# tensorlink-lab/tensorlink

Hardware: NVIDIA H100
Metric: generate tokens/sec (higher is better)
Workload: dtype bf16

## Files before the change

tensorlink_b200/csrc/attention.cu:

```cuda
#include <stdlib.h>

#include "common.cuh"

namespace tl {

constexpr int FA_BQ = 64, FA_BKV = 64, FA_THREADS = 128;

__device__ __forceinline__ void cp_async16(void* smem_dst, const void* gsrc, bool valid) {
    const uint32_t d = smem_u32(smem_dst);
    const int sz = valid ? 16 : 0;
    asm volatile("cp.async.cg.shared.global [%0], [%1], 16, %2;" ::"r"(d), "l"(gsrc), "r"(sz) : "memory");
}
__device__ __forceinline__ void cp_async_commit() { asm volatile("cp.async.commit_group;" ::: "memory"); }
template <int N>
__device__ __forceinline__ void cp_async_wait() { asm volatile("cp.async.wait_group %0;" ::"n"(N) : "memory"); }

__device__ __forceinline__ void ldmatrix_x4(uint32_t* r, const void* p) {
    asm volatile("ldmatrix.sync.aligned.m8n8.x4.shared.b16 {%0,%1,%2,%3}, [%4];"
                 : "=r"(r[0]), "=r"(r[1]), "=r"(r[2]), "=r"(r[3]) : "r"(smem_u32(p)));
}
__device__ __forceinline__ void ldmatrix_x4_trans(uint32_t* r, const void* p) {
    asm volatile("ldmatrix.sync.aligned.m8n8.x4.trans.shared.b16 {%0,%1,%2,%3}, [%4];"
                 : "=r"(r[0]), "=r"(r[1]), "=r"(r[2]), "=r"(r[3]) : "r"(smem_u32(p)));
}
// ... 584 lines not shown
                for (int ks = 0; ks < D / 16; ++ks)
                    ldmatrix_x4(qf[ks], sQ + (warp * 16 + (lane & 15)) * LDS + ks * 16 + (lane >> 4) * 8);
            }
            const bf16* sKb = sK + (t & 1) * FA_BKV * LDS;
            const bf16* sVb = sV + (t & 1) * FA_BKV * LDS;
            float s[FA_BKV / 8][4];
#pragma unroll
            for (int i = 0; i < FA_BKV / 8; ++i) s[i][0] = s[i][1] = s[i][2] = s[i][3] = 0.f;
#pragma unroll
            for (int ks = 0; ks < D / 16; ++ks) {
#pragma unroll
                for (int np = 0; np < FA_BKV / 16; ++np) {
                    uint32_t bfr[4];
                    const int mi = lane >> 3;
                    ldmatrix_x4(bfr, sKb + (np * 16 + (mi >> 1) * 8 + (lane & 7)) * LDS + ks * 16 + (mi & 1) * 8);
                    mma_bf16_16816(s[2 * np], qf[ks], bfr[0], bfr[1]);
                    mma_bf16_16816(s[2 * np + 1], qf[ks], bfr[2], bfr[3]);
                }
            }
            const int kv0 = c0 + t * FA_BKV;
            float mx[2] = {-INFINITY, -INFINITY};
#pragma unroll
            for (int i = 0; i < FA_BKV / 8; ++i) {
#pragma unroll
                for (int e = 0; e < 4; ++e) {
                    const int key = kv0 + i * 8 + 2 * t4 + (e & 1);
                    const float v = key <= last[e >> 1] ? s[i][e] * scale_log2 : -INFINITY;
                    s[i][e] = v;
                    mx[e >> 1] = fmaxf(mx[e >> 1], v);
                }
            }
            float alpha[2], msub[2];
#pragma unroll
            for (int r = 0; r < 2; ++r) {
                mx[r] = fmaxf(mx[r], __shfl_xor_sync(0xffffffffu, mx[r], 1));
                mx[r] = fmaxf(mx[r], __shfl_xor_sync(0xffffffffu, mx[r], 2));
                const float m_new = fmaxf(m_run[r], mx[r]);
                msub[r] = (m_new == -INFINITY) ? 0.f : m_new;
                alpha[r] = exp2f(m_run[r] - msub[r]);
                m_run[r] = m_new;
            }
            float rs[2] = {0.f, 0.f};
            uint32_t pf[FA_BKV / 16][4];
#pragma unroll
            for (int i = 0; i < FA_BKV / 8; ++i) {
                const float p0 = exp2f(s[i][0] - msub[0]), p1 = exp2f(s[i][1] - msub[0]);
                const float p2 = exp2f(s[i][2] - msub[1]), p3 = exp2f(s[i][3] - msub[1]);
                rs[0] += p0 + p1;
                rs[1] += p2 + p3;
                pf[i >> 1][(i & 1) * 2] = pack_bf16(p0, p1);
                pf[i >> 1][(i & 1) * 2 + 1] = pack_bf16(p2, p3);
            }
#pragma unroll
            for (int r = 0; r < 2; ++r) {
                rs[r] += __shfl_xor_sync(0xffffffffu, rs[r], 1);
                rs[r] += __shfl_xor_sync(0xffffffffu, rs[r], 2);
                l_run[r] = l_run[r] * alpha[r] + rs[r];
            }
#pragma unroll
            for (int i = 0; i < D / 8; ++i) {
                o[i][0] *= alpha[0];
                o[i][1] *= alpha[0];
                o[i][2] *= alpha[1];
                o[i][3] *= alpha[1];
            }
#pragma unroll
            for (int kk = 0; kk < FA_BKV / 16; ++kk) {
#pragma unroll
                for (int dp = 0; dp < D / 16; ++dp) {
                    uint32_t bfr[4];
                    const int mi = lane >> 3;
                    ldmatrix_x4_trans(bfr, sVb + (kk * 16 + (mi & 1) * 8 + (lane & 7)) * LDS + dp * 16 + (mi >> 1) * 8);
                    mma_bf16_16816(o[2 * dp], pf[kk], bfr[0], bfr[1]);
                    mma_bf16_16816(o[2 * dp + 1], pf[kk], bfr[2], bfr[3]);
                }
            }
        }
        if (t + 2 < n_tiles) {
            __syncthreads();
            load_tile(t + 2);
        }
    }
    if (!active) return;
#pragma unroll
    for (int r = 0; r < 2; ++r) {
        const int m = m0 + warp * 16 + g + r * 8;
        if (m >= M) continue;
        float* rec = ws + (((size_t)kvh * n_splits + split) * M + m) * (2 + D);
        if (t4 == 0) { rec[0] = m_run[r]; rec[1] = l_run[r]; }
#pragma unroll
        for (int i = 0; i < D / 8; ++i)
            *reinterpret_cast<float2*>(rec + 2 + i * 8 + 2 * t4) = make_float2(o[i][2 * r], o[i][2 * r + 1]);
    }
}

template <int D>
__global__ void attn_verify_reduce_kernel(const float* __restrict__ ws, bf16* __restrict__ out, const int32_t* __restrict__ pos_dev,
                                          int q_len, int n_h, int n_kv, int T_max, int n_splits) {
    const int h = blockIdx.x, i = blockIdx.y, dd = threadIdx.x;
    const int n_rep = n_h / n_kv, kvh = h / n_rep, M = n_rep * q_len, m = i * n_rep + (h - kvh * n_rep);
    const int last = min(*pos_dev + i, T_max - 1);
    const int ns = min(n_splits, last / DEC_CHUNK_MMA + 1);
    const float* base = ws + ((size_t)kvh * n_splits * M + m) * (2 + D);
    const size_t step = (size_t)M * (2 + D);
    float Mx = -INFINITY;
    for (int s = 0; s < ns; ++s) Mx = fmaxf(Mx, base[s * step]);
    float L = 0.f, O = 0.f;
    for (int s = 0; s < ns; ++s) {
        const float* rec = base + s * step;
        if (rec[0] == -INFINITY) continue;
        const float w = exp2f(rec[0] - Mx);
        L += rec[1] * w;
        O += rec[2 + dd] * w;
    }
    out[((size_t)i * n_h + h) * D + dd] = f2bf(L > 0.f ? O / L : 0.f);
}

}

namespace tl {
int attn_prefill_wgmma(const void* q, const void* k_cache, const void* v_cache, void* out, float* lse, int B, int S, int past_len,
                       int n_h, int n_kv, int d, int T_max, float scale, const int32_t* kv_start, cudaStream_t st);

static int attn_prefill_launch(const void* q, const void* k_cache, const void* v_cache, void* out, float* lse, int B, int S,
                               int past_len, int n_h, int n_kv, int d, int T_max, float scale, const int32_t* kv_start,
                               cudaStream_t st, const char* what) {
    TL_REQUIRE(d == 64 || d == 128, TL_ERR_INVALID, "%s: head_dim %d not in {64,128}", what, d);
    TL_REQUIRE(n_kv > 0 && n_h % n_kv == 0, TL_ERR_INVALID, "%s: n_h %% n_kv != 0", what);
    TL_REQUIRE(past_len >= 0 && past_len + S <= T_max, TL_ERR_INVALID,
               "%s: past_len %d + S %d exceeds cache T_max %d", what, past_len, S, T_max);
    if (B == 0 || S == 0) return TL_OK;
    {
        const char* e = getenv("TL_ATTN_IMPL");
        const int impl = !e ? 0 : (e[0] == 'm' ? 1 : (e[0] == 'w' ? 2 : 0));
        if (impl == 2 || (impl == 0 && S >= FA_BQ))
            return attn_prefill_wgmma(q, k_cache, v_cache, out, lse, B, S, past_len, n_h, n_kv, d, T_max, scale, kv_start, st);
    }
    const dim3 grid((S + FA_BQ - 1) / FA_BQ, n_h, B);
    const float sl2 = scale * 1.4426950408889634f;
    const size_t smem = (size_t)(FA_BQ + 4 * FA_BKV) * (d + 8) * sizeof(bf16);
#define TL_FA_FWD(D_, ROWS_)                                                                                                \
    do {                                                                                                                    \
        static bool done = false;                                                                                           \
        if (!done) { cudaFuncSetAttribute(attn_prefill_kernel<D_, ROWS_>, cudaFuncAttributeMaxDynamicSharedMemorySize, (int)smem); done = true; } \
        attn_prefill_kernel<D_, ROWS_><<<grid, FA_THREADS, smem, st>>>((const bf16*)q, (const bf16*)k_cache, (const bf16*)v_cache, \
                                                                        (bf16*)out, lse, S, past_len, n_h, n_kv, T_max, sl2, kv_start); \
    } while (0)
    if (kv_start) {
        if (d == 64) TL_FA_FWD(64, true); else TL_FA_FWD(128, true);
    } else {
        if (d == 64) TL_FA_FWD(64, false); else TL_FA_FWD(128, false);
    }
#undef TL_FA_FWD
    return check_launch(what);
}

static int attn_decode_launch(const void* q, const void* k_cache, const void* v_cache, void* out, const int32_t* kv_len_dev,
                              void* workspace, size_t ws_bytes, int B, int n_h, int n_kv, int d, int T_max, float scale,
                              const int32_t* kv_start, cudaStream_t st, const char* what);
}

extern "C" {

int tl_attn_prefill_fwd(const void* q, const void* k_cache, const void* v_cache, void* out, float* lse, int B, int S,
                        int past_len, int n_h, int n_kv, int d, int T_max, float scale, void* stream) {
    return tl::attn_prefill_launch(q, k_cache, v_cache, out, lse, B, S, past_len, n_h, n_kv, d, T_max, scale, nullptr,
                                   (cudaStream_t)stream, "tl_attn_prefill_fwd");
}

int tl_attn_prefill_fwd_rows(const void* q, const void* k_cache, const void* v_cache, void* out, float* lse, int B, int S,
                             int past_len, int n_h, int n_kv, int d, int T_max, float scale, const int32_t* kv_start_dev,
                             void* stream) {
    using namespace tl;
    TL_REQUIRE(kv_start_dev != nullptr, TL_ERR_INVALID, "tl_attn_prefill_fwd_rows: kv_start_dev is null");
    return attn_prefill_launch(q, k_cache, v_cache, out, lse, B, S, past_len, n_h, n_kv, d, T_max, scale, kv_start_dev,
                               (cudaStream_t)stream, "tl_attn_prefill_fwd_rows");
}

size_t tl_attn_decode_ws(int B, int n_h, int d, int T_max) {
    const size_t n_splits = (size_t)(T_max + tl::DEC_CHUNK - 1) / tl::DEC_CHUNK;
    return (size_t)B * n_splits * (size_t)n_h * (2 + d) * sizeof(float);
}

int tl_attn_decode_fwd(const void* q, const void* k_cache, const void* v_cache, void* out, const int32_t* kv_len_dev,
                       void* workspace, size_t ws_bytes, int B, int n_h, int n_kv, int d, int T_max, float scale,
                       void* stream) {
    return tl::attn_decode_launch(q, k_cache, v_cache, out, kv_len_dev, workspace, ws_bytes, B, n_h, n_kv, d, T_max, scale,
                                  nullptr, (cudaStream_t)stream, "tl_attn_decode_fwd");
}

int tl_attn_decode_fwd_rows(const void* q, const void* k_cache, const void* v_cache, void* out, const int32_t* kv_len_dev,
                            void* workspace, size_t ws_bytes, int B, int n_h, int n_kv, int d, int T_max, float scale,
                            const int32_t* kv_start_dev, void* stream) {
    using namespace tl;
    TL_REQUIRE(kv_start_dev != nullptr, TL_ERR_INVALID, "tl_attn_decode_fwd_rows: kv_start_dev is null");
    return attn_decode_launch(q, k_cache, v_cache, out, kv_len_dev, workspace, ws_bytes, B, n_h, n_kv, d, T_max, scale,
                              kv_start_dev, (cudaStream_t)stream, "tl_attn_decode_fwd_rows");
}

size_t tl_attn_verify_ws(int q_len, int n_h, int d, int T_max) {
    const size_t n_splits = (size_t)(T_max + tl::DEC_CHUNK_MMA - 1) / tl::DEC_CHUNK_MMA;
    return n_splits * (size_t)n_h * (size_t)(q_len > 0 ? q_len : 0) * (2 + d) * sizeof(float);
}

int tl_attn_verify_fwd(const void* q, const void* k_cache, const void* v_cache, void* out, const int32_t* pos_dev,
                       void* workspace, size_t ws_bytes, int q_len, int n_h, int n_kv, int d, int T_max, float scale,
                       void* stream) {
    using namespace tl;
    const char* what = "tl_attn_verify_fwd";
    TL_REQUIRE(d == 64 || d == 128, TL_ERR_INVALID, "%s: head_dim %d not in {64,128}", what, d);
    TL_REQUIRE(n_kv > 0 && n_h % n_kv == 0 && n_h / n_kv <= DEC_MAX_REP, TL_ERR_INVALID,
               "%s: GQA group %d/%d unsupported (max %d)", what, n_h, n_kv, DEC_MAX_REP);
    TL_REQUIRE(q_len >= 1 && q_len <= VER_MAX_Q, TL_ERR_INVALID, "%s: q_len %d not in [1, %d]", what, q_len, VER_MAX_Q);
    TL_REQUIRE(q && k_cache && v_cache && out && pos_dev && workspace, TL_ERR_INVALID, "%s: null argument", what);
    TL_REQUIRE(T_max >= q_len, TL_ERR_INVALID, "%s: T_max %d < q_len %d", what, T_max, q_len);
    TL_REQUIRE(ws_bytes >= tl_attn_verify_ws(q_len, n_h, d, T_max), TL_ERR_WORKSPACE,
               "%s: workspace %zu < %zu", what, ws_bytes, tl_attn_verify_ws(q_len, n_h, d, T_max));
    const int n_splits = (T_max + DEC_CHUNK_MMA - 1) / DEC_CHUNK_MMA;
    const int M = n_h / n_kv * q_len;
    const dim3 g1(n_splits, n_kv, (M + FA_BQ - 1) / FA_BQ), g2(n_h, q_len);
    const float sl2 = scale * 1.4426950408889634f;
    const size_t smem = (size_t)(FA_BQ + 4 * FA_BKV) * (d + 8) * sizeof(bf16);
    cudaStream_t st = (cudaStream_t)stream;
#define TL_VERIFY(D_)                                                                                                       \
    do {                                                                                                                    \
        static bool done = false;                                                                                           \
        if (!done) { cudaFuncSetAttribute(attn_verify_mma_kernel<D_>, cudaFuncAttributeMaxDynamicSharedMemorySize, (int)smem); done = true; } \
        attn_verify_mma_kernel<D_><<<g1, FA_THREADS, smem, st>>>((const bf16*)q, (const bf16*)k_cache, (const bf16*)v_cache,     \
                                                                 (float*)workspace, pos_dev, q_len, n_h, n_kv, T_max, n_splits, sl2); \
        attn_verify_reduce_kernel<D_><<<g2, D_, 0, st>>>((const float*)workspace, (bf16*)out, pos_dev, q_len, n_h, n_kv, T_max, \
                                                         n_splits);                                                         \
    } while (0)
    if (d == 64) TL_VERIFY(64); else TL_VERIFY(128);
#undef TL_VERIFY
    return check_launch(what);
}

}

namespace tl {
static int attn_decode_launch(const void* q, const void* k_cache, const void* v_cache, void* out, const int32_t* kv_len_dev,
                              void* workspace, size_t ws_bytes, int B, int n_h, int n_kv, int d, int T_max, float scale,
                              const int32_t* kv_start, cudaStream_t st, const char* what) {
    TL_REQUIRE(d == 64 || d == 128, TL_ERR_INVALID, "%s: head_dim %d not in {64,128}", what, d);
    TL_REQUIRE(n_kv > 0 && n_h % n_kv == 0 && n_h / n_kv <= DEC_MAX_REP, TL_ERR_INVALID,
               "%s: GQA group %d/%d unsupported (max %d)", what, n_h, n_kv, DEC_MAX_REP);
    TL_REQUIRE(kv_len_dev != nullptr, TL_ERR_INVALID, "%s: kv_len_dev is null", what);
    TL_REQUIRE(ws_bytes >= tl_attn_decode_ws(B, n_h, d, T_max), TL_ERR_WORKSPACE,
               "%s: workspace %zu < %zu", what, ws_bytes, tl_attn_decode_ws(B, n_h, d, T_max));
    if (B == 0) return TL_OK;
    const int n_splits = (T_max + DEC_CHUNK - 1) / DEC_CHUNK;
    const float sl2 = scale * 1.4426950408889634f;
    const dim3 g1(n_splits, n_kv, B), g2(n_h, B);
    const char* impl = getenv("TL_DECODE_ATTN");
    if (!(impl && impl[0] == 's')) {
        const int ns_m = (T_max + DEC_CHUNK_MMA - 1) / DEC_CHUNK_MMA;
        const dim3 gm(ns_m, n_kv, B);
        const size_t smem = (size_t)(16 + 4 * FA_BKV) * (d + 8) * sizeof(bf16);
#define TL_DEC_MMA(D_, ROWS_)                                                                                               \
        do {                                                                                                                \
            static bool done = false;                                                                                       \
            if (!done) { cudaFuncSetAttribute(attn_decode_mma_kernel<D_, ROWS_>, cudaFuncAttributeMaxDynamicSharedMemorySize, (int)smem); done = true; } \
            attn_decode_mma_kernel<D_, ROWS_><<<gm, FA_THREADS, smem, st>>>((const bf16*)q, (const bf16*)k_cache, (const bf16*)v_cache, \
                                                                             (float*)workspace, kv_len_dev, n_h, n_kv, T_max, ns_m, sl2, kv_start); \
            attn_decode_reduce_kernel<D_, ROWS_><<<g2, D_, 0, st>>>((const float*)workspace, (bf16*)out, kv_len_dev, n_h, n_kv, ns_m, \
                                                                     DEC_CHUNK_MMA, kv_start);                             \
        } while (0)
        if (kv_start) {
            if (d == 64) TL_DEC_MMA(64, true); else TL_DEC_MMA(128, true);
        } else {
            if (d == 64) TL_DEC_MMA(64, false); else TL_DEC_MMA(128, false);
        }
#undef TL_DEC_MMA
        return check_launch(what);
    }
#define TL_DEC_SIMT(D_, ROWS_)                                                                                              \
    do {                                                                                                                    \
        attn_decode_split_kernel<D_, ROWS_><<<g1, DEC_THREADS, 0, st>>>((const bf16*)q, (const bf16*)k_cache, (const bf16*)v_cache, \
                                                                         (float*)workspace, kv_len_dev, n_h, n_kv, T_max, n_splits, sl2, kv_start); \
        attn_decode_reduce_kernel<D_, ROWS_><<<g2, D_, 0, st>>>((const float*)workspace, (bf16*)out, kv_len_dev, n_h, n_kv, n_splits, \
                                                                 DEC_CHUNK, kv_start);                                     \
    } while (0)
    if (kv_start) {
        if (d == 64) TL_DEC_SIMT(64, true); else TL_DEC_SIMT(128, true);
    } else {
        if (d == 64) TL_DEC_SIMT(64, false); else TL_DEC_SIMT(128, false);
    }
#undef TL_DEC_SIMT
    return check_launch(what);
}
}

namespace tl {

constexpr int FD_THREADS = 128, FD_MAX_T = 2048;

template <int D, bool ROWS>
__global__ void __launch_bounds__(FD_THREADS) attn_decode_fused_kernel(
    const bf16* __restrict__ qkv, bf16* __restrict__ k_cache, bf16* __restrict__ v_cache, bf16* __restrict__ out,
    const int32_t* __restrict__ pos_dev, const bf16* __restrict__ cos_tab, const bf16* __restrict__ sin_tab,
    const bf16* __restrict__ q_norm_w, const bf16* __restrict__ k_norm_w, float eps, int n_h, int n_kv, int T_max,
    float scale_log2, const int32_t* __restrict__ kv_start) {
    constexpr int HALF = D / 2;
    asm volatile("griddepcontrol.wait;" ::: "memory");
    asm volatile("griddepcontrol.launch_dependents;");
    const int h = blockIdx.x, b = blockIdx.y, tid = threadIdx.x, lane = tid & 31, warp = tid >> 5;
    const int n_rep = n_h / n_kv, kvh = h / n_rep;
    const int pos = *pos_dev;
    int k_start = 0;
    if constexpr (ROWS) {
        k_start = kv_start[b];
        cos_tab -= (size_t)k_start * HALF;
        sin_tab -= (size_t)k_start * HALF;
    }
    const int heads = n_h + 2 * n_kv;
    __shared__ __align__(16) float sq[D], sk[D], sv[D];
    __shared__ float sscore[FD_MAX_T + 1];
    __shared__ float sred[FD_THREADS / 32];
    __shared__ float s_bc[2];
    __shared__ __align__(16) float so[FD_THREADS / 32][D];

    const bf16* row = qkv + (size_t)b * heads * D;
    float q1 = 0.f, q2 = 0.f, k1 = 0.f, k2 = 0.f;
    if (tid < HALF) {
        q1 = bf2f(row[(size_t)h * D + tid]);
        q2 = bf2f(row[(size_t)h * D + tid + HALF]);
        k1 = bf2f(row[(size_t)(n_h + kvh) * D + tid]);
        k2 = bf2f(row[(size_t)(n_h + kvh) * D + tid + HALF]);
        sv[tid] = bf2f(row[(size_t)(n_h + n_kv + kvh) * D + tid]);
        sv[tid + HALF] = bf2f(row[(size_t)(n_h + n_kv + kvh) * D + tid + HALF]);
    }
    if (q_norm_w) {
        float a = warp_sum(q1 * q1 + q2 * q2), c = warp_sum(k1 * k1 + k2 * k2);
        __shared__ float nr[2][FD_THREADS / 32];
        if (lane == 0) { nr[0][warp] = a; nr[1][warp] = c; }
        __syncthreads();
        a = c = 0.f;
#pragma unroll
        for (int w = 0; w < FD_THREADS / 32; ++w) { a += nr[0][w]; c += nr[1][w]; }
        const float rq = 1.0f / sqrtf(a / (float)D + eps), rk = 1.0f / sqrtf(c / (float)D + eps);
        if (tid < HALF) {
            q1 = rbf(bf2f(q_norm_w[tid]) * rbf(q1 * rq));
            q2 = rbf(bf2f(q_norm_w[tid + HALF]) * rbf(q2 * rq));
            k1 = rbf(bf2f(k_norm_w[tid]) * rbf(k1 * rk));
            k2 = rbf(bf2f(k_norm_w[tid + HALF]) * rbf(k2 * rk));
        }
    }
    if (tid < HALF) {
        const float c = bf2f(cos_tab[(size_t)pos * HALF + tid]), s = bf2f(sin_tab[(size_t)pos * HALF + tid]);
        sq[tid] = rbf(rbf(q1 * c) + rbf(-q2 * s));
        sq[tid + HALF] = rbf(rbf(q2 * c) + rbf(q1 * s));
        sk[tid] = rbf(rbf(k1 * c) + rbf(-k2 * s));
        sk[tid + HALF] = rbf(rbf(k2 * c) + rbf(k1 * s));
    }
    __syncthreads();
    if (h % n_rep == 0 && tid < D) {
        const size_t off = (((size_t)b * n_kv + kvh) * T_max + pos) * D + tid;
        k_cache[off] = f2bf(sk[tid]);
        v_cache[off] = f2bf(sv[tid]);
    }
    const bf16* kb = k_cache + ((size_t)b * n_kv + kvh) * T_max * D;
    const bf16* vb = v_cache + ((size_t)b * n_kv + kvh) * T_max * D;
    float mx = -INFINITY;
    for (int key = tid; key < pos; key += FD_THREADS) {
        if constexpr (ROWS) if (key < k_start) continue;
        const uint4* kr = reinterpret_cast<const uint4*>(kb + (size_t)key * D);
        float acc = 0.f;
#pragma unroll 4
        for (int c = 0; c < D / 8; ++c) {
            const uint4 kv4 = kr[c];
            const uint32_t* k32 = reinterpret_cast<const uint32_t*>(&kv4);
            const float4 qa = *reinterpret_cast<const float4*>(&sq[c * 8]);
            const float4 qb = *reinterpret_cast<const float4*>(&sq[c * 8 + 4]);
            acc += bf16_lo(k32[0]) * qa.x + bf16_hi(k32[0]) * qa.y + bf16_lo(k32[1]) * qa.z + bf16_hi(k32[1]) * qa.w +
                   bf16_lo(k32[2]) * qb.x + bf16_hi(k32[2]) * qb.y + bf16_lo(k32[3]) * qb.z + bf16_hi(k32[3]) * qb.w;
        }
        acc *= scale_log2;
        sscore[key] = acc;
        mx = fmaxf(mx, acc);
    }
    if (warp == 0) {
        float acc = 0.f;
        for (int i = lane; i < D; i += 32) acc += sq[i] * sk[i];
        acc = warp_sum(acc) * scale_log2;
        if (lane == 0) sscore[pos] = acc;
        mx = fmaxf(mx, acc);
    }
    mx = warp_max(mx);
    if (lane == 0) sred[warp] = mx;
    __syncthreads();
    if (tid == 0) {
        float m = sred[0];
#pragma unroll
        for (int w = 1; w < FD_THREADS / 32; ++w) m = fmaxf(m, sred[w]);
        s_bc[0] = m;
    }
    __syncthreads();
    const float m_all = s_bc[0];
    float lsum = 0.f;
    for (int key = tid; key <= pos; key += FD_THREADS) {
        if constexpr (ROWS) if (key < k_start) continue;
        const float p = exp2f(sscore[key] - m_all);
        lsum += p;
        sscore[key] = rbf(p);
    }
    lsum = warp_sum(lsum);
    __syncthreads();
    if (lane == 0) sred[warp] = lsum;
    __syncthreads();
    constexpr int TPR = D / 8, KG = FD_THREADS / TPR;
    const int dd0 = (tid % TPR) * 8, kgi = tid / TPR;
    float acc[8];
#pragma unroll
    for (int j = 0; j < 8; ++j) acc[j] = 0.f;
    for (int key = kgi; key < pos; key += KG) {
        if constexpr (ROWS) if (key < k_start) continue;
        const uint4 vv = *reinterpret_cast<const uint4*>(vb + (size_t)key * D + dd0);
        const uint32_t* v32 = reinterpret_cast<const uint32_t*>(&vv);
        const float p = sscore[key];
#pragma unroll
        for (int j = 0; j < 4; ++j) {
            acc[2 * j] = fmaf(p, bf16_lo(v32[j]), acc[2 * j]);
            acc[2 * j + 1] = fmaf(p, bf16_hi(v32[j]), acc[2 * j + 1]);
        }
    }
    if (kgi == 0) {
        const float p = sscore[pos];
#pragma unroll
        for (int j = 0; j < 8; ++j) acc[j] = fmaf(p, sv[dd0 + j], acc[j]);
    }
#pragma unroll
    for (int j = 0; j < 8; ++j) {
        float v = acc[j];
#pragma unroll
        for (int off = TPR; off < 32; off <<= 1) v += __shfl_xor_sync(0xffffffffu, v, off);
        acc[j] = v;
    }
    if (lane < TPR) {
#pragma unroll
        for (int j = 0; j < 8; ++j) so[warp][dd0 + j] = acc[j];
    }
    __syncthreads();
    if (tid < D) {
        float l = 0.f, o = 0.f;
#pragma unroll
        for (int w = 0; w < FD_THREADS / 32; ++w) { l += sred[w]; o += so[w][tid]; }
        out[((size_t)b * n_h + h) * D + tid] = f2bf(o / l);
    }
}

}

namespace tl {
static int attn_decode_fused_cfg(cudaLaunchConfig_t* cfg, cudaLaunchAttribute* attr, int d, int n_h, int n_kv, int T_max,
                                 const int32_t* pos_dev, int B, void* stream, const char* what) {
    TL_REQUIRE(d == 64 || d == 128, TL_ERR_INVALID, "%s: head_dim %d not in {64,128}", what, d);
    TL_REQUIRE(n_kv > 0 && n_h % n_kv == 0, TL_ERR_INVALID, "%s: n_h %% n_kv != 0", what);
    TL_REQUIRE(T_max <= FD_MAX_T, TL_ERR_INVALID, "%s: T_max %d > %d (use the split-KV path)", what, T_max, FD_MAX_T);
    TL_REQUIRE(pos_dev != nullptr, TL_ERR_INVALID, "%s: pos_dev is null", what);
    *cfg = {};
    cfg->gridDim = dim3(n_h, B);
    cfg->blockDim = dim3(FD_THREADS);
    cfg->dynamicSmemBytes = 0;
    cfg->stream = (cudaStream_t)stream;
    attr[0].id = cudaLaunchAttributeProgrammaticStreamSerialization;
    attr[0].val.programmaticStreamSerializationAllowed = 1;
    static int use_pdl = -1;
    if (use_pdl < 0) {
        const char* e = getenv("TL_PDL");
        const char* e2 = getenv("TL_PDL_ATTN");
        use_pdl = (!(e && e[0] == '0') && (e2 && e2[0] == '1')) ? 1 : 0;
    }
    cfg->attrs = attr;
    cfg->numAttrs = use_pdl ? 1 : 0;
    return TL_OK;
}
}

extern "C" int tl_attn_decode_fused(const void* qkv, void* k_cache, void* v_cache, void* out, const int32_t* pos_dev,
                                    const void* cos_tab, const void* sin_tab, const void* q_norm_w, const void* k_norm_w,
                                    float eps, int B, int n_h, int n_kv, int d, int T_max, float scale, void* stream) {
    using namespace tl;
    cudaLaunchConfig_t cfg;
    cudaLaunchAttribute attr[1];
    const int rc = attn_decode_fused_cfg(&cfg, attr, d, n_h, n_kv, T_max, pos_dev, B, stream, "tl_attn_decode_fused");
    if (rc != TL_OK || B == 0) return rc;
    const float sl2 = scale * 1.4426950408889634f;
    if (d == 64)
        cudaLaunchKernelEx(&cfg, attn_decode_fused_kernel<64, false>, (const bf16*)qkv, (bf16*)k_cache, (bf16*)v_cache, (bf16*)out,
                           pos_dev, (const bf16*)cos_tab, (const bf16*)sin_tab, (const bf16*)q_norm_w, (const bf16*)k_norm_w, eps,
                           n_h, n_kv, T_max, sl2, (const int32_t*)nullptr);
    else
        cudaLaunchKernelEx(&cfg, attn_decode_fused_kernel<128, false>, (const bf16*)qkv, (bf16*)k_cache, (bf16*)v_cache, (bf16*)out,
                           pos_dev, (const bf16*)cos_tab, (const bf16*)sin_tab, (const bf16*)q_norm_w, (const bf16*)k_norm_w, eps,
                           n_h, n_kv, T_max, sl2, (const int32_t*)nullptr);
    return check_launch("tl_attn_decode_fused");
}

extern "C" int tl_attn_decode_fused_rows(const void* qkv, void* k_cache, void* v_cache, void* out, const int32_t* pos_dev,
                                         const void* cos_tab, const void* sin_tab, const void* q_norm_w, const void* k_norm_w,
                                         float eps, int B, int n_h, int n_kv, int d, int T_max, float scale,
                                         const int32_t* kv_start_dev, void* stream) {
    using namespace tl;
    TL_REQUIRE(kv_start_dev != nullptr, TL_ERR_INVALID, "tl_attn_decode_fused_rows: kv_start_dev is null");
    cudaLaunchConfig_t cfg;
    cudaLaunchAttribute attr[1];
    const int rc = attn_decode_fused_cfg(&cfg, attr, d, n_h, n_kv, T_max, pos_dev, B, stream, "tl_attn_decode_fused_rows");
    if (rc != TL_OK || B == 0) return rc;
    const float sl2 = scale * 1.4426950408889634f;
    if (d == 64)
        cudaLaunchKernelEx(&cfg, attn_decode_fused_kernel<64, true>, (const bf16*)qkv, (bf16*)k_cache, (bf16*)v_cache, (bf16*)out,
                           pos_dev, (const bf16*)cos_tab, (const bf16*)sin_tab, (const bf16*)q_norm_w, (const bf16*)k_norm_w, eps,
                           n_h, n_kv, T_max, sl2, kv_start_dev);
    else
        cudaLaunchKernelEx(&cfg, attn_decode_fused_kernel<128, true>, (const bf16*)qkv, (bf16*)k_cache, (bf16*)v_cache, (bf16*)out,
                           pos_dev, (const bf16*)cos_tab, (const bf16*)sin_tab, (const bf16*)q_norm_w, (const bf16*)k_norm_w, eps,
                           n_h, n_kv, T_max, sl2, kv_start_dev);
    return check_launch("tl_attn_decode_fused_rows");
}
```

tensorlink_b200/csrc/gemv_stream.cu:

```cuda
#include <stdlib.h>

#include "common.cuh"

namespace tl {

constexpr int GS_CONSUMER_WARPS = 8;
constexpr int GS_THREADS = (GS_CONSUMER_WARPS + 1) * 32;
constexpr int GS_MAX_STAGES = 16;
constexpr int GS_STAGE_BYTES = 16 * 1024;
constexpr int GS_KC = 4096;
constexpr int GS_TICKET_BYTES = 24 * 1024;
constexpr int GS_SKIP = -2;
constexpr int GS_LEAVE = -1;

__device__ __forceinline__ void named_bar_sync(int id, int nthreads) {
    asm volatile("bar.sync %0, %1;" ::"r"(id), "r"(nthreads) : "memory");
}

template <int M>
__global__ void __launch_bounds__(GS_THREADS, 1)
gemv_stream_kernel(const bf16* __restrict__ x, const bf16* __restrict__ W, bf16* __restrict__ y, int N, int K,
                   const bf16* __restrict__ bias, const bf16* __restrict__ residual, const bf16* __restrict__ norm_w,
                   float eps, int flags, int P, int n_stages, int NW, int stage_bytes, int G, unsigned* __restrict__ ctr,
                   const unsigned char* __restrict__ pf_ptr, unsigned long long pf_bytes) {
    extern __shared__ __align__(128) unsigned char smem[];
    unsigned char* ring = smem;
    bf16* xs = reinterpret_cast<bf16*>(smem + (size_t)n_stages * stage_bytes);
    uint64_t* full_bar = reinterpret_cast<uint64_t*>(smem + (size_t)n_stages * stage_bytes + (((size_t)M * K * 2 + 15) & ~(size_t)15));
    uint64_t* empty_bar = full_bar + GS_MAX_STAGES;
    __shared__ float s_part[GS_CONSUMER_WARPS][M];
    __shared__ int s_unit[GS_MAX_STAGES];

    asm volatile("griddepcontrol.launch_dependents;");
    const int tid = threadIdx.x, lane = tid & 31, warp = tid >> 5;
    const int npairs = N >> 1;
    const int n_units = (npairs + P - 1) / P;
    const bool chunked = K > GS_KC || (size_t)K * 4 > GS_STAGE_BYTES;
    const int KC = chunked ? GS_KC : K;
    const int n_chunks = (K + KC - 1) / KC;

    if (tid == 0) {
        for (int s = 0; s < n_stages; ++s) {
            mbar_init(&full_bar[s], 1);
            mbar_init(&empty_bar[s], 1);
        }
        fence_barrier_init();
    }
    __syncthreads();

    if (warp == GS_CONSUMER_WARPS) {
        if (lane == 0) {
            const int first = gridDim.x * G;
            const bool tickets = first < n_units;
            int t_cur = blockIdx.x * G, t_used = 0;
            int t_next = tickets ? first + ticket_take(ctr, G) : n_units;
            auto next_unit = [&]() -> int {
                if (t_used == G) {
                    if (t_next >= n_units) return n_units;
                    t_cur = t_next;
                    t_used = 0;
                    t_next = first + ticket_take(ctr, G);
                }
                return t_cur + t_used++;
            };
            int unit[GS_CONSUMER_WARPS], chunk[GS_CONSUMER_WARPS], skip[GS_CONSUMER_WARPS];
#pragma unroll
            for (int w = 0; w < GS_CONSUMER_WARPS; ++w) {
                unit[w] = 0;
                chunk[w] = 0;
                skip[w] = chunked ? w * n_chunks / NW : 0;
            }
            int stage = 0, live = NW;
            uint32_t phase = 0;
            while (live > 0) {
#pragma unroll
                for (int w = 0; w < GS_CONSUMER_WARPS; ++w) {
                    if (w >= NW) continue;
                    if (unit[w] != GS_LEAVE) {
                        mbar_wait(&empty_bar[stage], phase ^ 1);
                        unsigned char* dst = ring + (size_t)stage * stage_bytes;
                        if (skip[w] > 0) {
                            --skip[w];
                            s_unit[stage] = GS_SKIP;
                            mbar_expect_tx(&full_bar[stage], 0);
                        } else {
                            if (chunk[w] == 0) {
                                unit[w] = next_unit();
                                if (unit[w] >= n_units) unit[w] = GS_LEAVE;
                            }
                            s_unit[stage] = unit[w];
                            if (unit[w] == GS_LEAVE) {
                                --live;
                                mbar_expect_tx(&full_bar[stage], 0);
                            } else if (!chunked) {
                                const int pair0 = unit[w] * P;
                                const int np = min(P, npairs - pair0);
                                const uint32_t bytes = (uint32_t)(2 * np) * (uint32_t)K * 2u;
                                mbar_expect_tx(&full_bar[stage], bytes);
                                bulk_load_1d(dst, W + (size_t)(2 * pair0) * K, bytes, &full_bar[stage]);
                            } else {
                                const int k0 = chunk[w] * KC;
                                const uint32_t bytes = (uint32_t)min(KC, K - k0) * 2u;
                                mbar_expect_tx(&full_bar[stage], 2 * bytes);
                                bulk_load_1d(dst, W + (size_t)(2 * unit[w]) * K + k0, bytes, &full_bar[stage]);
                                bulk_load_1d(dst + (size_t)KC * 2, W + (size_t)(2 * unit[w] + 1) * K + k0, bytes, &full_bar[stage]);
                                if (++chunk[w] == n_chunks) chunk[w] = 0;
                            }
                        }
                    }
                    if (++stage == n_stages) { stage = 0; phase ^= 1; }
                }
            }
            if (tickets && last_cta_out(ctr + 1)) {
                ctr[0] = 0u;
                __threadfence();
            }
            if (pf_bytes) {
                const unsigned long long per = ((pf_bytes / gridDim.x) + 4095ull) & ~4095ull;
                unsigned long long off = (unsigned long long)blockIdx.x * per;
                const unsigned long long end = off + per < pf_bytes ? off + per : pf_bytes;
                for (; off < end; off += 16384ull) {
                    const uint32_t sz = (uint32_t)(end - off < 16384ull ? end - off : 16384ull);
                    asm volatile("cp.async.bulk.prefetch.L2.global [%0], %1;" ::"l"(pf_ptr + off), "r"(sz) : "memory");
                }
            }
        }
    } else {
        asm volatile("griddepcontrol.wait;" ::: "memory");
        const int nvec = K >> 3;
        if (norm_w) {
            float ss[M];
#pragma unroll
            for (int m = 0; m < M; ++m) ss[m] = 0.f;
            for (int v = tid; v < nvec; v += GS_CONSUMER_WARPS * 32) {
#pragma unroll
                for (int m = 0; m < M; ++m) {
                    const uint4 u = reinterpret_cast<const uint4*>(x + (size_t)m * K)[v];
                    const uint32_t* u32 = reinterpret_cast<const uint32_t*>(&u);
#pragma unroll
                    for (int j = 0; j < 4; ++j) {
                        const float a = bf16_lo(u32[j]), b = bf16_hi(u32[j]);
                        ss[m] += a * a + b * b;
                    }
                }
            }
#pragma unroll
            for (int m = 0; m < M; ++m) {
                const float t = warp_sum(ss[m]);
                if (lane == 0) s_part[warp][m] = t;
            }
            named_bar_sync(1, GS_CONSUMER_WARPS * 32);
            float rstd[M];
#pragma unroll
            for (int m = 0; m < M; ++m) {
                float t = 0.f;
#pragma unroll
                for (int w = 0; w < GS_CONSUMER_WARPS; ++w) t += s_part[w][m];
                rstd[m] = 1.0f / sqrtf(t / (float)K + eps);
            }
            for (int v = tid; v < nvec; v += GS_CONSUMER_WARPS * 32) {
                const uint4 g = reinterpret_cast<const uint4*>(norm_w)[v];
                const uint32_t* g32 = reinterpret_cast<const uint32_t*>(&g);
#pragma unroll
                for (int m = 0; m < M; ++m) {
                    const uint4 u = reinterpret_cast<const uint4*>(x + (size_t)m * K)[v];
                    uint4 o;
                    const uint32_t* u32 = reinterpret_cast<const uint32_t*>(&u);
                    uint32_t* o32 = reinterpret_cast<uint32_t*>(&o);
#pragma unroll
                    for (int j = 0; j < 4; ++j)
                        o32[j] = pack_bf16(bf16_lo(g32[j]) * rbf(bf16_lo(u32[j]) * rstd[m]),
                                           bf16_hi(g32[j]) * rbf(bf16_hi(u32[j]) * rstd[m]));
                    reinterpret_cast<uint4*>(xs + (size_t)m * K)[v] = o;
                }
            }
        } else {
            for (int v = tid; v < nvec * M; v += GS_CONSUMER_WARPS * 32)
                reinterpret_cast<uint4*>(xs)[v] = reinterpret_cast<const uint4*>(x)[v];
        }
        named_bar_sync(1, GS_CONSUMER_WARPS * 32);

        const bool swiglu = flags & TL_EPI_SWIGLU;
        const int n_out = swiglu ? npairs : N;
        auto finish = [&](int pair, const float (&a0)[M], const float (&a1)[M]) {
            if (lane != 0) return;
            const int r0 = 2 * pair;
#pragma unroll
            for (int m = 0; m < M; ++m) {
                float v0 = a0[m], v1 = a1[m];
                if (flags & TL_EPI_BIAS) {
                    v0 += bf2f(bias[r0]);
                    v1 += bf2f(bias[r0 + 1]);
                }
                if (swiglu) {
                    const float gate = rbf(v0), up = rbf(v1);
                    y[(size_t)m * n_out + pair] = f2bf(rbf(silu_f(gate)) * up);
                } else {
                    float t0 = rbf(v0), t1 = rbf(v1);
                    if (flags & TL_EPI_RESIDUAL) {
                        t0 += bf2f(residual[(size_t)m * N + r0]);
                        t1 += bf2f(residual[(size_t)m * N + r0 + 1]);
                    }
                    *reinterpret_cast<uint32_t*>(y + (size_t)m * N + r0) = pack_bf16(t0, t1);
                }
            }
        };
        auto dot2 = [&](const uint4* r0, const uint4* r1, int k0, int vecs, float (&a0)[M], float (&a1)[M]) {
#pragma unroll 4
            for (int v = lane; v < vecs; v += 32) {
                const uint4 w0 = r0[v], w1 = r1[v];
                const uint32_t* a32 = reinterpret_cast<const uint32_t*>(&w0);
                const uint32_t* b32 = reinterpret_cast<const uint32_t*>(&w1);
#pragma unroll
                for (int m = 0; m < M; ++m) {
                    const uint4 xv = reinterpret_cast<const uint4*>(xs + (size_t)m * K + k0)[v];
                    const uint32_t* x32 = reinterpret_cast<const uint32_t*>(&xv);
#pragma unroll
                    for (int j = 0; j < 4; ++j) {
                        const float xl = bf16_lo(x32[j]), xh = bf16_hi(x32[j]);
                        a0[m] = fmaf(bf16_lo(a32[j]), xl, a0[m]);
                        a0[m] = fmaf(bf16_hi(a32[j]), xh, a0[m]);
                        a1[m] = fmaf(bf16_lo(b32[j]), xl, a1[m]);
                        a1[m] = fmaf(bf16_hi(b32[j]), xh, a1[m]);
                    }
                }
            }
        };
        int seq = warp, c = 0;
        float a0[M], a1[M];
#pragma unroll
        for (int m = 0; m < M; ++m) a0[m] = a1[m] = 0.f;
        while (warp < NW) {
            const int stage = seq % n_stages;
            const uint32_t phase = (uint32_t)(seq / n_stages) & 1u;
            mbar_wait(&full_bar[stage], phase);
            const int unit = s_unit[stage];
            if (unit == GS_LEAVE) break;
            const unsigned char* src = ring + (size_t)stage * stage_bytes;
            if (unit >= 0 && !chunked) {
                const int pair0 = unit * P;
                const int np = min(P, npairs - pair0);
                for (int pp = 0; pp < np; ++pp) {
                    float b0[M], b1[M];
#pragma unroll
                    for (int m = 0; m < M; ++m) b0[m] = b1[m] = 0.f;
                    dot2(reinterpret_cast<const uint4*>(src + (size_t)(2 * pp) * K * 2),
                         reinterpret_cast<const uint4*>(src + (size_t)(2 * pp + 1) * K * 2), 0, nvec, b0, b1);
#pragma unroll
                    for (int m = 0; m < M; ++m) { b0[m] = warp_sum(b0[m]); b1[m] = warp_sum(b1[m]); }
                    finish(pair0 + pp, b0, b1);
                }
            } else if (unit >= 0) {
                const int k0 = c * KC;
                dot2(reinterpret_cast<const uint4*>(src), reinterpret_cast<const uint4*>(src + (size_t)KC * 2), k0,
                     min(KC, K - k0) >> 3, a0, a1);
            }
            __syncwarp();
            if (lane == 0) mbar_arrive(&empty_bar[stage]);
            seq += NW;
            if (unit >= 0 && chunked && ++c == n_chunks) {
#pragma unroll
                for (int m = 0; m < M; ++m) { a0[m] = warp_sum(a0[m]); a1[m] = warp_sum(a1[m]); }
                finish(unit, a0, a1);
#pragma unroll
                for (int m = 0; m < M; ++m) a0[m] = a1[m] = 0.f;
                c = 0;
            }
        }
    }
}

template <int M>
static int launch_stream(const void* x, const void* W, void* y, int N, int K, const void* bias, const void* residual,
                         const void* norm_w, float eps, int flags, unsigned* ctr, const void* pf_ptr, size_t pf_bytes,
                         cudaStream_t st) {
    auto kern = gemv_stream_kernel<M>;
    static int forced = -1;
    if (forced < 0) {
        const char* e = getenv("TL_GEMV_CTAS_PER_SM");
        forced = (e && e[0] == '2') ? 2 : ((e && e[0] == '1') ? 1 : 0);
    }
    const int per_sm = forced ? forced : (((size_t)N * K * 2 / (size_t)sm_count() <= (size_t)128 * 1024) ? 2 : 1);
    static int ring_kb = 0;
    if (ring_kb == 0) {
        const char* e = getenv("TL_GEMV_RING_KB");
        ring_kb = e ? atoi(e) : 220;
        if (ring_kb < 48 || ring_kb > 220) ring_kb = 220;
    }
    const int SMEM_CAP = per_sm == 2 ? 110 * 1024 : ring_kb * 1024;
    static bool attr_done = false;
    if (!attr_done) {
        if (cudaFuncSetAttribute(kern, cudaFuncAttributeMaxDynamicSharedMemorySize, 220 * 1024) != cudaSuccess)
            return check_launch("tl_gemv_bf16/stream (smem attr)");
        attr_done = true;
    }
    const size_t xs_bytes = (((size_t)M * K * 2) + 15) & ~(size_t)15;
    const size_t fixed = xs_bytes + 2 * GS_MAX_STAGES * sizeof(uint64_t);
    const bool chunked = K > GS_KC || (size_t)K * 4 > GS_STAGE_BYTES;
    int P = chunked ? 1 : (int)(GS_STAGE_BYTES / ((size_t)K * 4));
    if (P < 1) P = 1;
    if (P > 8) P = 8;
    const int stage_bytes = chunked ? GS_STAGE_BYTES : (int)((((size_t)P * K * 4) + 127) & ~(size_t)127);
    int max_stages = (int)((SMEM_CAP - fixed) / stage_bytes);
    if (max_stages > GS_MAX_STAGES) max_stages = GS_MAX_STAGES;
    if (max_stages < 4) return 1;
    int n_stages = 0, NW = 0;
    for (int nw = GS_CONSUMER_WARPS; nw >= 4; --nw) {
        const int st_ = max_stages / nw * nw;
        if (st_ > n_stages) { n_stages = st_; NW = nw; }
    }
    const size_t smem = (size_t)n_stages * stage_bytes + fixed;
    const int npairs = N >> 1;
    int grid = sm_count() * per_sm;
    if (grid > npairs) grid = npairs;
    int G;
    if (npairs <= 8 * grid) {
        P = 1;
        G = (npairs + grid - 1) / grid;
    } else {
        const int unit_bytes = chunked ? K * 4 : P * K * 4;
        G = (GS_TICKET_BYTES + unit_bytes - 1) / unit_bytes;
    }
    cudaLaunchConfig_t cfg = {};
    cfg.gridDim = dim3(grid);
    cfg.blockDim = dim3(GS_THREADS);
    cfg.dynamicSmemBytes = smem;
    cfg.stream = st;
    cudaLaunchAttribute attr[1];
    attr[0].id = cudaLaunchAttributeProgrammaticStreamSerialization;
    attr[0].val.programmaticStreamSerializationAllowed = 1;
    static int use_pdl = -1;
    if (use_pdl < 0) {
        const char* e = getenv("TL_PDL");
        use_pdl = (e && e[0] == '0') ? 0 : 1;
    }
    cfg.attrs = attr;
    cfg.numAttrs = use_pdl ? 1 : 0;
    cudaLaunchKernelEx(&cfg, kern, (const bf16*)x, (const bf16*)W, (bf16*)y, N, K, (const bf16*)bias, (const bf16*)residual,
                       (const bf16*)norm_w, eps, flags, P, n_stages, NW, stage_bytes, G, ctr, (const unsigned char*)pf_ptr,
                       (unsigned long long)(pf_bytes & ~(size_t)15));
    return check_launch("tl_gemv_bf16/stream");
}

int gemv_stream_dispatch(const void* x, const void* W, void* y, int M, int N, int K, const void* bias,
                         const void* residual, const void* norm_w, float eps, int flags, unsigned* ctr, const void* pf_ptr,
                         size_t pf_bytes, cudaStream_t st) {
    if (K % 8 != 0 || ((uintptr_t)W & 15)) return 1;
    if ((uintptr_t)pf_ptr & 15) pf_bytes = 0;
    switch (M) {
        case 1: return launch_stream<1>(x, W, y, N, K, bias, residual, norm_w, eps, flags, ctr, pf_ptr, pf_bytes, st);
        case 2: return launch_stream<2>(x, W, y, N, K, bias, residual, norm_w, eps, flags, ctr, pf_ptr, pf_bytes, st);
        case 3: return launch_stream<3>(x, W, y, N, K, bias, residual, norm_w, eps, flags, ctr, pf_ptr, pf_bytes, st);
        case 4: return launch_stream<4>(x, W, y, N, K, bias, residual, norm_w, eps, flags, ctr, pf_ptr, pf_bytes, st);
        default: return 1;
    }
}

}
```

Before: 202.7.

## Prefetch KV before PDL wait, enable attention PDL, relay chunked GEMV partials across warps

The decode attention kernel now issues L2 prefetches of the KV cache rows and rope tables before griddepcontrol.wait, and enables PDL by default, so KV loading can overlap the previous kernel's tail. The score buffer moves to dynamic shared memory sized by T_max. The streaming GEMV changes chunked K handling: chunks are balanced to multiples of 256, and a relay mode hands per-warp partial accumulators to the next warp through shared-memory mbarriers instead of having each warp skip ahead. This adds cross-warp synchronisation and shared-memory use. The prefetch also competes for bandwidth with the previous kernel while it is still running.

Result: no change. 203.8 (median of 6 runs) (+0.5%).

```diff
diff --git a/tensorlink_b200/csrc/attention.cu b/tensorlink_b200/csrc/attention.cu
--- a/tensorlink_b200/csrc/attention.cu
+++ b/tensorlink_b200/csrc/attention.cu
@@ -910,10 +910,28 @@
     const bf16* __restrict__ q_norm_w, const bf16* __restrict__ k_norm_w, float eps, int n_h, int n_kv, int T_max,
     float scale_log2, const int32_t* __restrict__ kv_start) {
     constexpr int HALF = D / 2;
+    const int h = blockIdx.x, b = blockIdx.y, tid = threadIdx.x, lane = tid & 31, warp = tid >> 5;
+    const int n_rep = n_h / n_kv, kvh = h / n_rep;
+    {
+        const int p = min(max(*pos_dev, 0), T_max - 1);
+        int ks = 0;
+        if constexpr (ROWS) ks = min(max(kv_start[b], 0), p);
+        const size_t rows = (size_t)(p - ks) * D * sizeof(bf16);
+        const size_t base = (((size_t)b * n_kv + kvh) * T_max + ks) * D;
+        const char* kp = reinterpret_cast<const char*>(k_cache + base);
+        const char* vp = reinterpret_cast<const char*>(v_cache + base);
+        const size_t stride = (size_t)n_rep * FD_THREADS * 128;
+        for (size_t off = ((size_t)(h % n_rep) * FD_THREADS + tid) * 128; off < rows; off += stride) {
+            asm volatile("prefetch.global.L2 [%0];" ::"l"(kp + off));
+            asm volatile("prefetch.global.L2 [%0];" ::"l"(vp + off));
+        }
+        if (tid == 0 && h % n_rep == 0) {
+            asm volatile("prefetch.global.L2 [%0];" ::"l"(cos_tab + (size_t)(p - ks) * HALF));
+            asm volatile("prefetch.global.L2 [%0];" ::"l"(sin_tab + (size_t)(p - ks) * HALF));
+        }
+    }
     asm volatile("griddepcontrol.wait;" ::: "memory");
     asm volatile("griddepcontrol.launch_dependents;");
-    const int h = blockIdx.x, b = blockIdx.y, tid = threadIdx.x, lane = tid & 31, warp = tid >> 5;
-    const int n_rep = n_h / n_kv, kvh = h / n_rep;
     const int pos = *pos_dev;
     int k_start = 0;
     if constexpr (ROWS) {
@@ -923,7 +941,7 @@
     }
     const int heads = n_h + 2 * n_kv;
     __shared__ __align__(16) float sq[D], sk[D], sv[D];
-    __shared__ float sscore[FD_MAX_T + 1];
+    extern __shared__ float sscore[];
     __shared__ float sred[FD_THREADS / 32];
     __shared__ float s_bc[2];
     __shared__ __align__(16) float so[FD_THREADS / 32][D];
@@ -1069,15 +1087,14 @@
     *cfg = {};
     cfg->gridDim = dim3(n_h, B);
     cfg->blockDim = dim3(FD_THREADS);
-    cfg->dynamicSmemBytes = 0;
+    cfg->dynamicSmemBytes = (size_t)(T_max + 1) * sizeof(float);
     cfg->stream = (cudaStream_t)stream;
     attr[0].id = cudaLaunchAttributeProgrammaticStreamSerialization;
     attr[0].val.programmaticStreamSerializationAllowed = 1;
     static int use_pdl = -1;
     if (use_pdl < 0) {
         const char* e = getenv("TL_PDL");
-        const char* e2 = getenv("TL_PDL_ATTN");
-        use_pdl = (!(e && e[0] == '0') && (e2 && e2[0] == '1')) ? 1 : 0;
+        use_pdl = (e && e[0] == '0') ? 0 : 1;
     }
     cfg->attrs = attr;
     cfg->numAttrs = use_pdl ? 1 : 0;
diff --git a/tensorlink_b200/csrc/gemv_stream.cu b/tensorlink_b200/csrc/gemv_stream.cu
--- a/tensorlink_b200/csrc/gemv_stream.cu
+++ b/tensorlink_b200/csrc/gemv_stream.cu
@@ -13,6 +13,12 @@
 constexpr int GS_SKIP = -2;
 constexpr int GS_LEAVE = -1;
 
+static inline int gs_chunk_len(int K) {
+    if (K <= GS_KC) return 0;
+    const int n = (K + GS_KC - 1) / GS_KC, groups = (K + 255) / 256;
+    return (groups + n - 1) / n * 256;
+}
+
 __device__ __forceinline__ void named_bar_sync(int id, int nthreads) {
     asm volatile("bar.sync %0, %1;" ::"r"(id), "r"(nthreads) : "memory");
 }
@@ -21,28 +27,38 @@
 __global__ void __launch_bounds__(GS_THREADS, 1)
 gemv_stream_kernel(const bf16* __restrict__ x, const bf16* __restrict__ W, bf16* __restrict__ y, int N, int K,
                    const bf16* __restrict__ bias, const bf16* __restrict__ residual, const bf16* __restrict__ norm_w,
-                   float eps, int flags, int P, int n_stages, int NW, int stage_bytes, int G, unsigned* __restrict__ ctr,
-                   const unsigned char* __restrict__ pf_ptr, unsigned long long pf_bytes) {
+                   float eps, int flags, int P, int n_stages, int NW, int stage_bytes, int KC, int relay, int G,
+                   unsigned* __restrict__ ctr, const unsigned char* __restrict__ pf_ptr, unsigned long long pf_bytes) {
     extern __shared__ __align__(128) unsigned char smem[];
     unsigned char* ring = smem;
     bf16* xs = reinterpret_cast<bf16*>(smem + (size_t)n_stages * stage_bytes);
     uint64_t* full_bar = reinterpret_cast<uint64_t*>(smem + (size_t)n_stages * stage_bytes + (((size_t)M * K * 2 + 15) & ~(size_t)15));
     uint64_t* empty_bar = full_bar + GS_MAX_STAGES;
+    uint64_t* hand_full = empty_bar + GS_MAX_STAGES;
+    uint64_t* hand_empty = hand_full + GS_CONSUMER_WARPS;
+    float* hand = reinterpret_cast<float*>(hand_empty + GS_CONSUMER_WARPS);
     __shared__ float s_part[GS_CONSUMER_WARPS][M];
     __shared__ int s_unit[GS_MAX_STAGES];
+    __shared__ int s_chunk[GS_MAX_STAGES];
 
     asm volatile("griddepcontrol.launch_dependents;");
     const int tid = threadIdx.x, lane = tid & 31, warp = tid >> 5;
     const int npairs = N >> 1;
     const int n_units = (npairs + P - 1) / P;
-    const bool chunked = K > GS_KC || (size_t)K * 4 > GS_STAGE_BYTES;
-    const int KC = chunked ? GS_KC : K;
+    const bool chunked = KC > 0;
+    if (!chunked) KC = K;
     const int n_chunks = (K + KC - 1) / KC;
 
     if (tid == 0) {
         for (int s = 0; s < n_stages; ++s) {
             mbar_init(&full_bar[s], 1);
             mbar_init(&empty_bar[s], 1);
+        }
+        if (relay) {
+            for (int w = 0; w < NW; ++w) {
+                mbar_init(&hand_full[w], 1);
+                mbar_init(&hand_empty[w], 1);
+            }
         }
         fence_barrier_init();
     }
@@ -64,19 +80,22 @@
                 return t_cur + t_used++;
             };
             int unit[GS_CONSUMER_WARPS], chunk[GS_CONSUMER_WARPS], skip[GS_CONSUMER_WARPS];
+            bool left[GS_CONSUMER_WARPS];
 #pragma unroll
             for (int w = 0; w < GS_CONSUMER_WARPS; ++w) {
                 unit[w] = 0;
                 chunk[w] = 0;
-                skip[w] = chunked ? w * n_chunks / NW : 0;
-            }
+                skip[w] = chunked && !relay ? w * n_chunks / NW : 0;
+                left[w] = false;
+            }
+            int r_unit = 0, r_chunk = 0;
             int stage = 0, live = NW;
             uint32_t phase = 0;
             while (live > 0) {
 #pragma unroll
                 for (int w = 0; w < GS_CONSUMER_WARPS; ++w) {
                     if (w >= NW) continue;
-                    if (unit[w] != GS_LEAVE) {
+                    if (!left[w]) {
                         mbar_wait(&empty_bar[stage], phase ^ 1);
                         unsigned char* dst = ring + (size_t)stage * stage_bytes;
                         if (skip[w] > 0) {
@@ -84,28 +103,32 @@
                             s_unit[stage] = GS_SKIP;
                             mbar_expect_tx(&full_bar[stage], 0);
                         } else {
-                            if (chunk[w] == 0) {
-                                unit[w] = next_unit();
-                                if (unit[w] >= n_units) unit[w] = GS_LEAVE;
+                            int u = relay ? r_unit : unit[w], c = relay ? r_chunk : chunk[w];
+                            if (c == 0 && u != GS_LEAVE) {
+                                u = next_unit();
+                                if (u >= n_units) u = GS_LEAVE;
                             }
-                            s_unit[stage] = unit[w];
-                            if (unit[w] == GS_LEAVE) {
+                            s_unit[stage] = u;
+                            s_chunk[stage] = c;
+                            if (u == GS_LEAVE) {
+                                left[w] = true;
                                 --live;
                                 mbar_expect_tx(&full_bar[stage], 0);
                             } else if (!chunked) {
-                                const int pair0 = unit[w] * P;
+                                const int pair0 = u * P;
                                 const int np = min(P, npairs - pair0);
                                 const uint32_t bytes = (uint32_t)(2 * np) * (uint32_t)K * 2u;
                                 mbar_expect_tx(&full_bar[stage], bytes);
                                 bulk_load_1d(dst, W + (size_t)(2 * pair0) * K, bytes, &full_bar[stage]);
                             } else {
-                                const int k0 = chunk[w] * KC;
+                                const int k0 = c * KC;
                                 const uint32_t bytes = (uint32_t)min(KC, K - k0) * 2u;
                                 mbar_expect_tx(&full_bar[stage], 2 * bytes);
-                                bulk_load_1d(dst, W + (size_t)(2 * unit[w]) * K + k0, bytes, &full_bar[stage]);
-                                bulk_load_1d(dst + (size_t)KC * 2, W + (size_t)(2 * unit[w] + 1) * K + k0, bytes, &full_bar[stage]);
-                                if (++chunk[w] == n_chunks) chunk[w] = 0;
+                                bulk_load_1d(dst, W + (size_t)(2 * u) * K + k0, bytes, &full_bar[stage]);
+                                bulk_load_1d(dst + (size_t)KC * 2, W + (size_t)(2 * u + 1) * K + k0, bytes, &full_bar[stage]);
+                                if (++c == n_chunks) c = 0;
                             }
+                            if (relay) { r_unit = u; r_chunk = c; } else { unit[w] = u; chunk[w] = c; }
                         }
                     }
                     if (++stage == n_stages) { stage = 0; phase ^= 1; }
@@ -227,6 +250,7 @@
             }
         };
         int seq = warp, c = 0;
+        uint32_t n_recv = 0, n_sent = 0;
         float a0[M], a1[M];
 #pragma unroll
         for (int m = 0; m < M; ++m) a0[m] = a1[m] = 0.f;
@@ -251,6 +275,15 @@
                     finish(pair0 + pp, b0, b1);
                 }
             } else if (unit >= 0) {
+                c = s_chunk[stage];
+                if (relay && c > 0) {
+                    mbar_wait(&hand_full[warp - 1], n_recv++ & 1u);
+                    const float* hp = hand + (size_t)(warp - 1) * 2 * M * 32 + lane;
+#pragma unroll
+                    for (int m = 0; m < M; ++m) { a0[m] = hp[(2 * m) * 32]; a1[m] = hp[(2 * m + 1) * 32]; }
+                    __syncwarp();
+                    if (lane == 0) mbar_arrive(&hand_empty[warp - 1]);
+                }
                 const int k0 = c * KC;
                 dot2(reinterpret_cast<const uint4*>(src), reinterpret_cast<const uint4*>(src + (size_t)KC * 2), k0,
                      min(KC, K - k0) >> 3, a0, a1);
@@ -258,13 +291,24 @@
             __syncwarp();
             if (lane == 0) mbar_arrive(&empty_bar[stage]);
             seq += NW;
-            if (unit >= 0 && chunked && ++c == n_chunks) {
-#pragma unroll
-                for (int m = 0; m < M; ++m) { a0[m] = warp_sum(a0[m]); a1[m] = warp_sum(a1[m]); }
-                finish(unit, a0, a1);
-#pragma unroll
-                for (int m = 0; m < M; ++m) a0[m] = a1[m] = 0.f;
-                c = 0;
+            if (unit >= 0 && chunked) {
+                if (c == n_chunks - 1) {
+#pragma unroll
+                    for (int m = 0; m < M; ++m) { a0[m] = warp_sum(a0[m]); a1[m] = warp_sum(a1[m]); }
+                    finish(unit, a0, a1);
+                } else if (relay) {
+                    if (n_sent > 0) mbar_wait(&hand_empty[warp], (n_sent - 1) & 1u);
+                    float* hp = hand + (size_t)warp * 2 * M * 32 + lane;
+#pragma unroll
+                    for (int m = 0; m < M; ++m) { hp[(2 * m) * 32] = a0[m]; hp[(2 * m + 1) * 32] = a1[m]; }
+                    ++n_sent;
+                    __syncwarp();
+                    if (lane == 0) mbar_arrive(&hand_full[warp]);
+                }
+                if (c == n_chunks - 1 || relay) {
+#pragma unroll
+                    for (int m = 0; m < M; ++m) a0[m] = a1[m] = 0.f;
+                }
             }
         }
     }
@@ -295,8 +339,9 @@
         attr_done = true;
     }
     const size_t xs_bytes = (((size_t)M * K * 2) + 15) & ~(size_t)15;
-    const size_t fixed = xs_bytes + 2 * GS_MAX_STAGES * sizeof(uint64_t);
-    const bool chunked = K > GS_KC || (size_t)K * 4 > GS_STAGE_BYTES;
+    const int KC = gs_chunk_len(K);
+    const bool chunked = KC > 0;
+    const size_t fixed = xs_bytes + 2 * GS_MAX_STAGES * sizeof(uint64_t) + (chunked ? 2 * GS_CONSUMER_WARPS * sizeof(uint64_t) : 0);
     int P = chunked ? 1 : (int)(GS_STAGE_BYTES / ((size_t)K * 4));
     if (P < 1) P = 1;
     if (P > 8) P = 8;
@@ -309,7 +354,20 @@
         const int st_ = max_stages / nw * nw;
         if (st_ > n_stages) { n_stages = st_; NW = nw; }
     }
-    const size_t smem = (size_t)n_stages * stage_bytes + fixed;
+    int relay = 0;
+    size_t hand_bytes = 0;
+    if (chunked) {
+        const int n_chunks = (K + KC - 1) / KC;
+        for (int nw = GS_CONSUMER_WARPS / n_chunks * n_chunks; nw >= n_chunks && nw > 0; nw -= n_chunks) {
+            const size_t hb = (size_t)nw * 2 * M * 32 * sizeof(float);
+            if (fixed + hb >= (size_t)SMEM_CAP) continue;
+            int ms = (int)((SMEM_CAP - fixed - hb) / stage_bytes);
+            if (ms > GS_MAX_STAGES) ms = GS_MAX_STAGES;
+            const int st_ = ms / nw * nw;
+            if (st_ >= n_stages && (!relay || st_ > n_stages)) { n_stages = st_; NW = nw; relay = 1; hand_bytes = hb; }
+        }
+    }
+    const size_t smem = (size_t)n_stages * stage_bytes + fixed + hand_bytes;
     const int npairs = N >> 1;
     int grid = sm_count() * per_sm;
     if (grid > npairs) grid = npairs;
@@ -337,7 +395,7 @@
     cfg.attrs = attr;
     cfg.numAttrs = use_pdl ? 1 : 0;
     cudaLaunchKernelEx(&cfg, kern, (const bf16*)x, (const bf16*)W, (bf16*)y, N, K, (const bf16*)bias, (const bf16*)residual,
-                       (const bf16*)norm_w, eps, flags, P, n_stages, NW, stage_bytes, G, ctr, (const unsigned char*)pf_ptr,
+                       (const bf16*)norm_w, eps, flags, P, n_stages, NW, stage_bytes, KC, relay, G, ctr, (const unsigned char*)pf_ptr,
                        (unsigned long long)(pf_bytes & ~(size_t)15));
     return check_launch("tl_gemv_bf16/stream");
 }
```
